# Penguin-jpg/clip-diffusion

Hardware: NVIDIA B200
Metric: CLIP-guided cutouts/s fwd+bwd inside full guidance steps (= steps/s x cutouts per step) @512x512 (higher is better)
Workload: dtype bf16

## Files before the change

clip_diffusion_b200/csrc/vit_attention_tc.cu:

```cuda
#include <stdlib.h>
#include "common.cuh"
#include "tcgen05.cuh"

using namespace tc;

namespace {

constexpr int AT_THREADS = 512;
constexpr int MAX_BLK = 5;
constexpr float LOG2E_F = 1.4426950408889634f;
constexpr uint32_t BLK_BYTES = 64 * 128;
constexpr uint32_t TILE_BYTES = 128 * 128;

__device__ __forceinline__ uint32_t pack_bf2(float a, float b) {
  __nv_bfloat162 v = __floats2bfloat162_rn(a, b);
  return *reinterpret_cast<uint32_t*>(&v);
}
__device__ __forceinline__ float ex2f(float x) {
  float y;
  asm("ex2.approx.ftz.f32 %0, %1;" : "=f"(y) : "f"(x));
  return y;
}
__device__ __forceinline__ float warp_max_f(float v) {
#pragma unroll
  for (int o = 16; o > 0; o >>= 1) v = fmaxf(v, __shfl_xor_sync(0xffffffffu, v, o));
  return v;
}
__device__ __forceinline__ void tmem_ld16(uint32_t taddr, uint32_t* r) {
  asm volatile(
      "tcgen05.ld.sync.aligned.32x32b.x16.b32 {%0, %1, %2, %3, %4, %5, %6, %7, %8, %9, %10, %11, %12, %13, %14, %15}, [%16];"
      : "=r"(r[0]), "=r"(r[1]), "=r"(r[2]), "=r"(r[3]), "=r"(r[4]), "=r"(r[5]), "=r"(r[6]), "=r"(r[7]), "=r"(r[8]), "=r"(r[9]), "=r"(r[10]),
        "=r"(r[11]), "=r"(r[12]), "=r"(r[13]), "=r"(r[14]), "=r"(r[15])
      : "r"(taddr)
      : "memory");
}
__device__ __forceinline__ uint32_t elect_one() {
  uint32_t pred;
  asm volatile("{\n\t.reg .pred P;\n\telect.sync _|P, 0xffffffff;\n\tselp.u32 %0, 1, 0, P;\n\t}" : "=r"(pred));
  return pred;
}
__device__ __forceinline__ uint32_t idesc_bf16(int n, bool b_mn_major) {
  return (1u << 4) | (1u << 7) | (1u << 10) | (b_mn_major ? (1u << 16) : 0u) | ((uint32_t)(n >> 3) << 17) | ((uint32_t)(128 >> 4) << 24);
}
__device__ __forceinline__ void st_shared_v4(uint32_t a, uint32_t x, uint32_t y, uint32_t z, uint32_t w) {
  asm volatile("st.shared.v4.b32 [%0], {%1, %2, %3, %4};" ::"r"(a), "r"(x), "r"(y), "r"(z), "r"(w) : "memory");
}
__device__ __forceinline__ void st256g(void* p, const uint32_t* w) {
  asm volatile("st.global.v8.b32 [%0], {%1,%2,%3,%4,%5,%6,%7,%8};" ::"l"(p), "r"(w[0]), "r"(w[1]), "r"(w[2]), "r"(w[3]), "r"(w[4]), "r"(w[5]),
               "r"(w[6]), "r"(w[7])
               : "memory");
}
__device__ __forceinline__ void store_row64_bf16(__nv_bfloat16* dst, const uint32_t* a, const uint32_t* b, float mul) {
  uint32_t w[32];
#pragma unroll
  for (int j = 0; j < 16; ++j) {
    w[j] = pack_bf2(__uint_as_float(a[2 * j]) * mul, __uint_as_float(a[2 * j + 1]) * mul);
    w[16 + j] = pack_bf2(__uint_as_float(b[2 * j]) * mul, __uint_as_float(b[2 * j + 1]) * mul);
  }
#pragma unroll
  for (int j = 0; j < 4; ++j) st256g(dst + 16 * j, w + 8 * j);
}

__device__ __forceinline__ uint32_t lds32(uint32_t a) {
  uint32_t v;
  asm volatile("ld.shared.b32 %0, [%1];" : "=r"(v) : "r"(a) : "memory");
  return v;
}
__device__ __forceinline__ float bf_lo(uint32_t u) { return __uint_as_float(u << 16); }
__device__ __forceinline__ float bf_hi(uint32_t u) { return __uint_as_float(u & 0xffff0000u); }
__device__ __forceinline__ float dot8p(const uint4 a, const uint4 b, float acc) {
  acc = fmaf(bf_lo(a.x), bf_lo(b.x), acc); acc = fmaf(bf_hi(a.x), bf_hi(b.x), acc); acc = fmaf(bf_lo(a.y), bf_lo(b.y), acc); acc = fmaf(bf_hi(a.y), bf_hi(b.y), acc);
  acc = fmaf(bf_lo(a.z), bf_lo(b.z), acc); acc = fmaf(bf_hi(a.z), bf_hi(b.z), acc); acc = fmaf(bf_lo(a.w), bf_lo(b.w), acc); acc = fmaf(bf_hi(a.w), bf_hi(b.w), acc);
  return acc;
}

struct AttnParams {
  int T, heads, ntiles, nblk, tail_rows;
  int nitems;
  int edge, nblk_ld, ld_tail;
  float scale;
  __nv_bfloat16* ctx;
  float* lse;
  const __nv_bfloat16* ctx_in;
  const __nv_bfloat16* dctx_in;
  __nv_bfloat16* dqkv;
  long long* trace;
};

struct FBars {
  uint32_t base;
  __device__ __forceinline__ uint32_t sfull(int b) const { return base + 8u * b; }
  __device__ __forceinline__ uint32_t sfree(int b) const { return base + 32u + 8u * b; }
  __device__ __forceinline__ uint32_t pready(int b) const { return base + 64u + 8u * b; }
  __device__ __forceinline__ uint32_t pfree(int b) const { return base + 96u + 8u * b; }
  __device__ __forceinline__ uint32_t accfull(int a) const { return base + 128u + 8u * a; }
  __device__ __forceinline__ uint32_t accfree(int a) const { return base + 160u + 8u * a; }
  __device__ __forceinline__ uint32_t mready(int a, uint32_t r) const { return base + 192u + 8u * (2u * a + r); }
  __device__ __forceinline__ uint32_t opq(int blk) const { return base + 256u + 8u * blk; }
  __device__ __forceinline__ uint32_t opk(int blk) const { return base + 296u + 8u * blk; }
  __device__ __forceinline__ uint32_t opv(int vb, int blk) const { return base + 336u + 8u * (vb * MAX_BLK + blk); }
  __device__ __forceinline__ uint32_t qkfree() const { return base + 416u; }
  __device__ __forceinline__ uint32_t vfree(int vb) const { return base + 424u + 8u * vb; }
  __device__ __forceinline__ uint32_t tmem_slot() const { return base + 440u; }
};
constexpr uint32_t FBARS_BYTES = 448 + 16;
constexpr uint32_t FWD_FLOATS = 4096 + 1024;
constexpr float RESCALE_LOG2 = 8.f;

__device__ __forceinline__ void tmem_st32(uint32_t taddr, const uint32_t* r) {
  asm volatile(
      "tcgen05.st.sync.aligned.32x32b.x32.b32 [%0], "
      "{%1, %2, %3, %4, %5, %6, %7, %8, %9, %10, %11, %12, %13, %14, %15, %16, "
      "%17, %18, %19, %20, %21, %22, %23, %24, %25, %26, %27, %28, %29, %30, %31, %32};" ::"r"(taddr),
      "r"(r[0]), "r"(r[1]), "r"(r[2]), "r"(r[3]), "r"(r[4]), "r"(r[5]), "r"(r[6]), "r"(r[7]), "r"(r[8]), "r"(r[9]), "r"(r[10]), "r"(r[11]), "r"(r[12]),
      "r"(r[13]), "r"(r[14]), "r"(r[15]), "r"(r[16]), "r"(r[17]), "r"(r[18]), "r"(r[19]), "r"(r[20]), "r"(r[21]), "r"(r[22]), "r"(r[23]), "r"(r[24]),
      "r"(r[25]), "r"(r[26]), "r"(r[27]), "r"(r[28]), "r"(r[29]), "r"(r[30]), "r"(r[31])
      : "memory");
}
__device__ __forceinline__ void tmem_st16(uint32_t taddr, const uint32_t* r) {
  asm volatile(
      "tcgen05.st.sync.aligned.32x32b.x16.b32 [%0], {%1, %2, %3, %4, %5, %6, %7, %8, %9, %10, %11, %12, %13, %14, %15, %16};" ::"r"(taddr),
      "r"(r[0]), "r"(r[1]), "r"(r[2]), "r"(r[3]), "r"(r[4]), "r"(r[5]), "r"(r[6]), "r"(r[7]), "r"(r[8]), "r"(r[9]), "r"(r[10]), "r"(r[11]), "r"(r[12]),
      "r"(r[13]), "r"(r[14]), "r"(r[15])
      : "memory");
}
// ... 555 lines not shown
      if (lane == 0) mbar_arrive(bars.vfree(vb));
    };
    float se0 = -INFINITY, se1 = -INFINITY, nse0 = -INFINITY, nse1 = -INFINITY;
    if ((int)blockIdx.x < nitems) { edge_a(blockIdx.x, 0, se0, se1); edge_b(blockIdx.x, 0); }
    int it = 0, gg0 = 0;
    for (int w = blockIdx.x; w < nitems; w += gridDim.x, ++it, gg0 += G) {
      const int n = w / heads, h = w - n * heads, row0 = n * T;
      const float* vedge = vedge2 + (it & 1) * 64;
      TRF(warp, 62, 0);
      TRI(warp, 0);
      for (int tile = 0; tile < ntiles; ++tile) {
        const int tp = tile & 1, a0 = tp, a1 = 2 + tp;
        const int ggt = gg0 + tile * nblk;
        const bool has0 = nblk > 1 || (ggt & 1) == 0, has1 = nblk > 1 || (ggt & 1) == 1;
        const uint32_t u0 = (euse >> (4 * a0)) & 15u, u1 = (euse >> (4 * a1)) & 15u;
        if (has0) { mbar_wait(bars.mready(a0, u0 & 1u), (u0 >> 1) & 1u); mbar_wait(bars.accfull(a0), u0 & 1u); }
        if (has1) { mbar_wait(bars.mready(a1, u1 & 1u), (u1 >> 1) & 1u); mbar_wait(bars.accfull(a1), u1 & 1u); }
        TRF(warp, tile, 0);
        tcgen05_fence_after();
        const int row = tile * 128 + rl;
        if (tile * 128 + q * 32 < Tp) {
          const float m0 = has0 ? sm[(a0 * 4 + (int)(u0 & 3u)) * 128 + rl] : -INFINITY, m1 = has1 ? sm[(a1 * 4 + (int)(u1 & 3u)) * 128 + rl] : -INFINITY;
          const float l0 = has0 ? sl[(a0 * 4 + (int)(u0 & 3u)) * 128 + rl] : 0.f, l1 = has1 ? sl[(a1 * 4 + (int)(u1 & 3u)) * 128 + rl] : 0.f;
          const float se = tile == 0 ? se0 : se1;
          const float M = fmaxf(fmaxf(m0, m1), se);
          const float f0 = has0 ? ex2f(m0 - M) : 0.f, f1 = has1 ? ex2f(m1 - M) : 0.f, fe = ex2f(se - M);
          const float L = l0 * f0 + l1 * f1 + fe;
          const float invL = __fdividef(1.f, L);
          const float g0 = f0 * invL, g1 = f1 * invL, ge = fe * invL;
          __nv_bfloat16* dst = p.ctx + ((long long)(row0 + row)) * D + h * 64;
#pragma unroll
          for (int c = 0; c < 64; c += 32) {
            uint32_t v0[32], v1[32], wv[16];
            if (has0) tmem_ld32(t_lane + 256u + (uint32_t)(a0 * 64 + c), v0);
            if (has1) tmem_ld32(t_lane + 256u + (uint32_t)(a1 * 64 + c), v1);
            tmem_ld_wait();
#pragma unroll
            for (int j = 0; j < 16; ++j) {
              float x0 = (has0 ? __uint_as_float(v0[2 * j]) * g0 : 0.f) + (has1 ? __uint_as_float(v1[2 * j]) * g1 : 0.f);
              float x1 = (has0 ? __uint_as_float(v0[2 * j + 1]) * g0 : 0.f) + (has1 ? __uint_as_float(v1[2 * j + 1]) * g1 : 0.f);
              if (edge) {
                const float2 ve = *reinterpret_cast<const float2*>(vedge + c + 2 * j);
                x0 = fmaf(ge, ve.x, x0);
                x1 = fmaf(ge, ve.y, x1);
              }
              wv[j] = pack_bf2(x0, x1);
            }
            if (row < Tp) { st256g(dst + c, wv); st256g(dst + c + 16, wv + 8); }
          }
          if (row < Tp) p.lse[((long long)n * heads + h) * T + row] = M * (1.f / LOG2E_F) + logf(L);
        }
        tcgen05_fence_before();
        __syncwarp();
        if (lane == 0) {
          if (has0) mbar_arrive(bars.accfree(a0));
          if (has1) mbar_arrive(bars.accfree(a1));
        }
        if (has0) euse = (euse & ~(15u << (4 * a0))) | (((u0 + 1u) & 15u) << (4 * a0));
        if (has1) euse = (euse & ~(15u << (4 * a1))) | (((u1 + 1u) & 15u) << (4 * a1));
        TRF(warp, tile, 1);
        if (tile == 0 && w + (int)gridDim.x < nitems) {
          TRF(warp, 61, 0);
          edge_a(w + gridDim.x, it + 1, nse0, nse1);
          edge_b(w + gridDim.x, it + 1);
          TRF(warp, 61, 1);
        }
      }
      se0 = nse0;
      se1 = nse1;
      TRF(warp, 62, 1);
      TRI(warp, 1);
    }
  }
  tcgen05_fence_before();
  __syncthreads();
  if (warp == 2) {
    tcgen05_fence_after();
    asm volatile("tcgen05.dealloc.cta_group::1.sync.aligned.b32 %0, %1;" ::"r"(tmem_base), "r"(512) : "memory");
  }
}

struct BBars {
  uint32_t base;
  __device__ __forceinline__ uint32_t sfull(int b) const { return base + 8u * b; }
  __device__ __forceinline__ uint32_t sfree(int b) const { return base + 24u + 8u * b; }
  __device__ __forceinline__ uint32_t pready(int pb) const { return base + 48u + 8u * pb; }
  __device__ __forceinline__ uint32_t pfree(int pb) const { return base + 64u + 8u * pb; }
  __device__ __forceinline__ uint32_t accfull(int a) const { return base + 80u + 8u * a; }
  __device__ __forceinline__ uint32_t accfree(int a) const { return base + 104u + 8u * a; }
  __device__ __forceinline__ uint32_t op(int o, int blk) const { return base + 128u + 8u * (o * MAX_BLK + blk); }
  __device__ __forceinline__ uint32_t opfree() const { return base + 288u; }
  __device__ __forceinline__ uint32_t cready(int par) const { return base + 296u + 8u * par; }
  __device__ __forceinline__ uint32_t tmem_slot() const { return base + 312u; }
};
constexpr uint32_t BBARS_BYTES = 320 + 16;
constexpr uint32_t BWD_FLOATS = 1280 + 1152 + 192 + 768;

#ifdef CG_ATTN_TRACE
#define TRB(slot, idx, ev) TRF(slot, idx, ev)
#else
#define TRB(slot, idx, ev) do { } while (0)
#endif

__device__ __forceinline__ void store_row64_bf16_axpy(__nv_bfloat16* dst, const uint32_t* a, const uint32_t* b, float coef, const float* vec) {
  uint32_t w[32];
#pragma unroll
  for (int j = 0; j < 16; ++j) {
    const float2 v0 = *reinterpret_cast<const float2*>(vec + 2 * j), v1 = *reinterpret_cast<const float2*>(vec + 32 + 2 * j);
    w[j] = pack_bf2(fmaf(coef, v0.x, __uint_as_float(a[2 * j])), fmaf(coef, v0.y, __uint_as_float(a[2 * j + 1])));
    w[16 + j] = pack_bf2(fmaf(coef, v1.x, __uint_as_float(b[2 * j])), fmaf(coef, v1.y, __uint_as_float(b[2 * j + 1])));
  }
#pragma unroll
  for (int j = 0; j < 4; ++j) st256g(dst + 16 * j, w + 8 * j);
}

__global__ void __launch_bounds__(AT_THREADS, 1)
    attn_bwd_tc_kernel(const __grid_constant__ CUtensorMap tmQKV, const __grid_constant__ CUtensorMap tmQKVtail, const __grid_constant__ CUtensorMap tmDO,
                       const __grid_constant__ CUtensorMap tmDOtail, const AttnParams p) {
  extern __shared__ __align__(1024) uint8_t smem_raw[];
  cg_griddep_launch();
  constexpr int NSB = 3;
  constexpr uint32_t STAGE_BYTES = 2 * TILE_BYTES;
  const int T = p.T, heads = p.heads, D = heads * 64;
  const int edge = p.edge, Tp = T - edge;
  const int warp = threadIdx.x >> 5, lane = threadIdx.x & 31;
  const int ntiles = p.ntiles, nblk = p.nblk, nblk_ld = p.nblk_ld;
  const int per_phase = ntiles * nblk, G = 2 * per_phase, nitems = p.nitems;
  const uint32_t opb = (uint32_t)((nblk_ld - 1) * 64 + p.ld_tail) * 128u;
  const uint32_t base = (smem_u32(smem_raw) + 1023u) & ~1023u;
  const uint32_t sOp0 = base;
  const uint32_t sStage = base + 4 * opb;
  const uint32_t sF = sStage + 2 * STAGE_BYTES;
  float* fscr = reinterpret_cast<float*>(smem_raw + (sF - smem_u32(smem_raw)));
  float* csts = fscr;
  float* ev = fscr + 1280;
  float* evec = fscr + 2432;
  float* epart = fscr + 2624;
  BBars bars{sF + BWD_FLOATS * 4};

  if (warp == 0 && lane == 0) {
    asm volatile("prefetch.tensormap [%0];" ::"l"(&tmQKV) : "memory");
    asm volatile("prefetch.tensormap [%0];" ::"l"(&tmQKVtail) : "memory");
    asm volatile("prefetch.tensormap [%0];" ::"l"(&tmDO) : "memory");
    asm volatile("prefetch.tensormap [%0];" ::"l"(&tmDOtail) : "memory");
    for (int b = 0; b < 3; ++b) {
      mbar_init(bars.sfull(b), 2); mbar_init(bars.sfree(b), 4);
      mbar_init(bars.accfull(b), 2); mbar_init(bars.accfree(b), 4);
    }
    for (int b = 0; b < 2; ++b) { mbar_init(bars.pready(b), 4); mbar_init(bars.pfree(b), 2); mbar_init(bars.cready(b), 4); }
    for (int o = 0; o < 4; ++o)
      for (int k = 0; k < MAX_BLK; ++k) mbar_init(bars.op(o, k), 1);
    mbar_init(bars.opfree(), 8);
    asm volatile("fence.mbarrier_init.release.cluster;" ::: "memory");
  }
  if (warp == 2) {
    asm volatile("tcgen05.alloc.cta_group::1.sync.aligned.shared::cta.b32 [%0], %1;" ::"r"(bars.tmem_slot()), "r"(512) : "memory");
    asm volatile("tcgen05.relinquish_alloc_permit.cta_group::1.sync.aligned;" ::: "memory");
  }
  cg_griddep_wait();
  tcgen05_fence_before();
  __syncthreads();
  tcgen05_fence_after();
  uint32_t tmem_base;
  asm volatile("ld.shared.b32 %0, [%1];" : "=r"(tmem_base) : "r"(bars.tmem_slot()) : "memory");

  if (warp < 4) {
    const uint32_t elected = elect_one();
    const uint32_t id_full = idesc_bf16(64, false), id_tail = idesc_bf16(p.tail_rows, false), id_acc = idesc_bf16(64, true);
    uint32_t cuse = 0;
    int it = 0, gg0 = 0;
    for (int w = blockIdx.x; w < nitems; w += gridDim.x, ++it, gg0 += G) {
      const uint32_t opar = (uint32_t)it & 1u;
      uint32_t loaded = 0;
      auto need = [&](int o, int blk) {
        const uint32_t bit = 1u << (o * MAX_BLK + blk);
        if (!(loaded & bit)) { mbar_wait(bars.op(o, blk), opar); loaded |= bit; }
      };
      if (warp == 3) {
        if (elected) {
          if (it > 0) mbar_wait(bars.opfree(), (uint32_t)(it - 1) & 1u);
          const int n = w / heads, h = w - n * heads, row0 = n * T;
          auto load = [&](int o, int blk) {
            const bool tail = blk == nblk_ld - 1;
            const uint32_t bar = bars.op(o, blk);
            mbar_arrive_expect_tx(bar, (uint32_t)(tail ? p.ld_tail : 64) * 128u);
            if (o < 3) tma_load_2d(sOp0 + o * opb + blk * BLK_BYTES, tail ? &tmQKVtail : &tmQKV, bar, o * D + h * 64, row0 + blk * 64);
            else tma_load_2d(sOp0 + o * opb + blk * BLK_BYTES, tail ? &tmDOtail : &tmDO, bar, h * 64, row0 + blk * 64);
          };
          const int first = nblk_ld < 2 ? nblk_ld : 2;
          load(1, 0);
#pragma unroll 1
          for (int k = 0; k < first; ++k) load(0, k);
          load(2, 0);
#pragma unroll 1
          for (int k = 0; k < first; ++k) load(3, k);
#pragma unroll 1
          for (int k = 1; k < nblk_ld; ++k) { load(1, k); load(2, k); }
#pragma unroll 1
          for (int k = first; k < nblk_ld; ++k) { load(0, k); load(3, k); }
          if (w + (int)gridDim.x < nitems) {
            const int w2 = w + gridDim.x, n2 = w2 / heads, h2 = w2 - n2 * heads;
#pragma unroll 1
            for (int k = 0; k < nblk_ld; ++k) {
              const bool tail = k == nblk_ld - 1;
#pragma unroll 1
              for (int o = 0; o < 3; ++o) tma_prefetch_2d(tail ? &tmQKVtail : &tmQKV, o * D + h2 * 64, n2 * T + k * 64);
              tma_prefetch_2d(tail ? &tmDOtail : &tmDO, h2 * 64, n2 * T + k * 64);
            }
          }
        }
        __syncwarp();
      }
      int phase = 0, tile = 0, blk = 0;
      if (warp < 2) {
        for (int g = 0; g < G; ++g) {
          const int gg = gg0 + g, b = gg % NSB;
          const bool transposed = phase == 1;
          const int oa = warp == 0 ? (transposed ? 1 : 0) : (transposed ? 2 : 3);
          const int ob = warp == 0 ? (transposed ? 0 : 1) : (transposed ? 3 : 2);
          need(oa, 2 * tile);
          if (2 * tile + 1 < nblk) need(oa, 2 * tile + 1);
          need(ob, blk);
          mbar_wait(bars.sfree(b), ((uint32_t)(gg / NSB) & 1u) ^ 1u);
          TRB(warp, g, 0);
          tcgen05_fence_after();
          const uint32_t d_s = tmem_base + (uint32_t)(b * 128) + (warp == 1 ? 64u : 0u);
          const uint64_t ad = make_smem_desc(sOp0 + oa * opb + tile * TILE_BYTES), bd = make_smem_desc(sOp0 + ob * opb + blk * BLK_BYTES);
          const uint32_t idesc = blk == nblk - 1 ? id_tail : id_full;
          if (elected) {
#pragma unroll
            for (int k = 0; k < 4; ++k) umma_bf16(d_s, ad + (uint64_t)(2 * k), bd + (uint64_t)(2 * k), idesc, k != 0 ? 1u : 0u);
            umma_commit(bars.sfull(b));
          }
          __syncwarp();
          TRB(warp, g, 1);
          if (++blk == nblk) { blk = 0; if (++tile == ntiles) { tile = 0; ++phase; } }
        }
      } else {
        const int wi = warp - 2;
        for (int g = 0; g < G; ++g) {
          const int gg = gg0 + g, pb = gg & 1;
          const int a = phase == 1 ? 2 : (tile & 1);
          const bool does_mma = phase == 1 || wi == 0;
          const int ob = phase == 0 ? 1 : (wi == 0 ? 3 : 0);
          if (does_mma) need(ob, blk);
          mbar_wait(bars.pready(pb), (uint32_t)(gg >> 1) & 1u);
          TRB(warp, g, 0);
          if (blk == 0) {
            if (phase == 1) {
              mbar_wait(bars.accfree(2), ((cuse >> 2) & 1u) ^ 1u);
              if (tile == 0) { mbar_wait(bars.accfree(0), (cuse & 1u) ^ 1u); mbar_wait(bars.accfree(1), ((cuse >> 1) & 1u) ^ 1u); }
            } else {
              mbar_wait(bars.accfree(a), ((cuse >> a) & 1u) ^ 1u);
              mbar_wait(bars.accfree(2), ((cuse >> 2) & 1u) ^ 1u);
            }
          }
          tcgen05_fence_after();
          const int ksteps = (blk == nblk - 1 ? p.tail_rows : 64) >> 4;
          const uint32_t stage = sStage + pb * STAGE_BYTES + (wi == 1 ? TILE_BYTES : 0u);
          const uint32_t d_acc = tmem_base + (a == 2 ? 384u : 384u + 64u * a) + (wi == 1 ? 64u : 0u);
          const uint64_t ad = make_smem_desc(stage), bd = make_smem_desc(sOp0 + ob * opb + blk * BLK_BYTES);
          const bool last = blk == nblk - 1;
          if (elected) {
            if (does_mma) {
              for (int k = 0; k < ksteps; ++k) umma_bf16(d_acc, ad + (uint64_t)(2 * k), bd + (uint64_t)(128 * k), id_acc, (blk | k) != 0 ? 1u : 0u);
              umma_commit(bars.pfree(pb));
              if (last) umma_commit(bars.accfull(a));
            } else {
              mbar_arrive(bars.pfree(pb));
              if (last) mbar_arrive(bars.accfull(a));
            }
          }
          __syncwarp();
          TRB(warp, g, 1);
          if (last) cuse ^= 1u << a;
          if (++blk == nblk) { blk = 0; if (++tile == ntiles) { tile = 0; ++phase; } }
        }
      }
#pragma unroll 1
      for (int o = 0; o < 4; ++o)
#pragma unroll 1
        for (int k = 0; k < nblk_ld; ++k) need(o, k);
      if (elected) umma_commit(bars.opfree());
      __syncwarp();
    }
  } else if (warp < 12) {
    const int wg = (warp - 4) >> 2;
    const int q = warp & 3;
    const int rl = q * 32 + lane;
    const uint32_t t_lane = tmem_base + ((uint32_t)(q * 32) << 16);
    const float scale = p.scale, sl2 = p.scale * LOG2E_F;
    const int tail_cols = Tp - (nblk - 1) * 64, tail_cols16 = p.tail_rows;
    const uint32_t sx = (uint32_t)(rl & 7) << 4;
    int it = 0, gg0 = 0;
    for (int w = blockIdx.x; w < nitems; w += gridDim.x, ++it, gg0 += G) {
      mbar_wait(bars.cready(it & 1), (uint32_t)(it >> 1) & 1u);
      const float* cst = csts + (it & 1) * 640;
      float rc0 = 0.f, rc1 = 0.f;
      int phase = 0, tile = 0, blk = wg, cur_tile = -1;
      while (blk >= nblk) { blk -= nblk; if (++tile == ntiles) { tile = 0; ++phase; } }
      for (int g = wg; g < G; g += 2) {
        const int gg = gg0 + g;
        if (phase == 0 && tile != cur_tile) {
          const int row = tile * 128 + rl;
          rc0 = row < Tp ? cst[row] : 0.f;
          rc1 = row < Tp ? cst[320 + row] : 0.f;
          cur_tile = tile;
        }
        const bool wvalid = tile * 128 + q * 32 < Tp;
        const bool tail = blk == nblk - 1;
        const int ncols = tail ? tail_cols : 64, ncols16 = tail ? tail_cols16 : 64;
        const int b = gg % NSB, pb = gg & 1;
        const uint32_t suse = (uint32_t)(gg / NSB), puse = (uint32_t)(gg >> 1);
        TRB(warp, g, 0);
        mbar_wait(bars.sfull(b), suse & 1u);
        TRB(warp, g, 1);
        tcgen05_fence_after();
        const uint32_t t_s = t_lane + (uint32_t)(b * 128);
        const uint32_t stage = sStage + pb * STAGE_BYTES + (uint32_t)rl * 128u;
        if (!wvalid) {
          tcgen05_fence_before();
          __syncwarp();
          if (lane == 0) mbar_arrive(bars.sfree(b));
          mbar_wait(bars.pfree(pb), (puse & 1u) ^ 1u);
        } else {
          uint32_t sv[2][16], dv[2][16], w0[8], w1[8];
          const int npieces = ncols16 >> 4;
          tmem_ld16(t_s, sv[0]);
          tmem_ld16(t_s + 64u, dv[0]);
          tmem_ld_wait();
          bool waited = false;
#pragma unroll
          for (int pc = 0; pc < 4; ++pc) {
            if (pc < npieces) {
              const int cur = pc & 1;
              if (pc + 1 < npieces) {
                tmem_ld16(t_s + (uint32_t)(16 * (pc + 1)), sv[cur ^ 1]);
                tmem_ld16(t_s + 64u + (uint32_t)(16 * (pc + 1)), dv[cur ^ 1]);
              }
              if (phase == 0) {
#pragma unroll
                for (int j = 0; j < 8; ++j) {
                  float p0 = ex2f(fmaf(__uint_as_float(sv[cur][2 * j]), sl2, rc0)), p1 = ex2f(fmaf(__uint_as_float(sv[cur][2 * j + 1]), sl2, rc0));
                  if (tail) { if (16 * pc + 2 * j >= ncols) p0 = 0.f; if (16 * pc + 2 * j + 1 >= ncols) p1 = 0.f; }
                  w0[j] = pack_bf2(p0 * fmaf(__uint_as_float(dv[cur][2 * j]), scale, rc1), p1 * fmaf(__uint_as_float(dv[cur][2 * j + 1]), scale, rc1));
                }
              } else {
                const float* nl = cst + blk * 64 + 16 * pc;
                const float* dl = nl + 320;
#pragma unroll
                for (int j = 0; j < 8; ++j) {
                  const float2 l2 = *reinterpret_cast<const float2*>(nl + 2 * j), d2 = *reinterpret_cast<const float2*>(dl + 2 * j);
                  float p0 = ex2f(fmaf(__uint_as_float(sv[cur][2 * j]), sl2, l2.x)), p1 = ex2f(fmaf(__uint_as_float(sv[cur][2 * j + 1]), sl2, l2.y));
                  if (tail) { if (16 * pc + 2 * j >= ncols) p0 = 0.f; if (16 * pc + 2 * j + 1 >= ncols) p1 = 0.f; }
                  w0[j] = pack_bf2(p0, p1);
                  w1[j] = pack_bf2(p0 * fmaf(__uint_as_float(dv[cur][2 * j]), scale, d2.x), p1 * fmaf(__uint_as_float(dv[cur][2 * j + 1]), scale, d2.y));
                }
              }
              if (!waited) { mbar_wait(bars.pfree(pb), (puse & 1u) ^ 1u); waited = true; }
              {
                const uint32_t c0 = ((uint32_t)(pc * 32)) ^ sx, c1 = ((uint32_t)(pc * 32 + 16)) ^ sx;
                st_shared_v4(stage + c0, w0[0], w0[1], w0[2], w0[3]);
                st_shared_v4(stage + c1, w0[4], w0[5], w0[6], w0[7]);
                if (phase == 1) {
                  st_shared_v4(stage + TILE_BYTES + c0, w1[0], w1[1], w1[2], w1[3]);
                  st_shared_v4(stage + TILE_BYTES + c1, w1[4], w1[5], w1[6], w1[7]);
                }
              }
              if (pc + 1 < npieces) {
                tmem_ld_wait();
              } else {
                tcgen05_fence_before();
                __syncwarp();
                if (lane == 0) mbar_arrive(bars.sfree(b));
              }
            }
          }
        }
        TRB(warp, g, 2);
        fence_proxy_async_smem();
        __syncwarp();
        if (lane == 0) mbar_arrive(bars.pready(pb));
        TRB(warp, g, 3);
        blk += 2;
        while (blk >= nblk) { blk -= nblk; if (++tile == ntiles) { tile = 0; ++phase; } }
      }
    }
  } else {
    const int q = warp & 3;
    const int rl = q * 32 + lane;
    const uint32_t t_lane = tmem_base + ((uint32_t)(q * 32) << 16);
    const float scale = p.scale, sl2 = p.scale * LOG2E_F;
    uint32_t euse = 0;
    auto load_consts = [&](int item, int par) {
      const int n = item / heads, h = item - n * heads;
      const float* lb = p.lse + ((long long)n * heads + h) * T;
      const __nv_bfloat16* ob = p.ctx_in + ((long long)n * T) * D + h * 64;
      const __nv_bfloat16* gb = p.dctx_in + ((long long)n * T) * D + h * 64;
      float* c = csts + par * 640;
      for (int i = rl; i < 320; i += 128) {
        float dl = 0.f, nl = -INFINITY;
        if (i < T) {
          const uint4* o4 = reinterpret_cast<const uint4*>(ob + (long long)i * D);
          const uint4* g4 = reinterpret_cast<const uint4*>(gb + (long long)i * D);
          uint4 xo[8], xg[8];
#pragma unroll
          for (int k = 0; k < 8; ++k) { xo[k] = __ldg(o4 + k); xg[k] = __ldg(g4 + k); }
          float d0 = 0.f, d1 = 0.f;
#pragma unroll
          for (int k = 0; k < 8; k += 2) { d0 = dot8p(xo[k], xg[k], d0); d1 = dot8p(xo[k + 1], xg[k + 1], d1); }
          dl = d0 + d1;
          nl = -lb[i] * LOG2E_F;
        }
        c[i] = nl;
        c[320 + i] = -p.scale * dl;
      }
      __syncwarp();
      if (lane == 0) mbar_arrive(bars.cready(par));
    };
    if ((int)blockIdx.x < nitems) load_consts(blockIdx.x, 0);
    int it = 0;
    for (int w = blockIdx.x; w < nitems; w += gridDim.x, ++it) {
      const int n = w / heads, h = w - n * heads, row0 = n * T;
      const uint32_t opar = (uint32_t)it & 1u;
      if (w + (int)gridDim.x < nitems) load_consts(w + gridDim.x, (it + 1) & 1);
      const float* cst = csts + (it & 1) * 640;
      __nv_bfloat16* out = p.dqkv + ((long long)row0) * 3 * D + h * 64;
      TRB(warp, 62, 0);
      TRI(warp, 0);
      if (edge) {
        for (int o = 0; o < 4; ++o)
          for (int k = 0; k < nblk_ld; ++k) mbar_wait(bars.op(o, k), opar);
        mbar_wait(bars.cready(it & 1), (uint32_t)(it >> 1) & 1u);
        TRB(warp, 61, 0);
        const uint32_t sQ = sOp0, sK = sOp0 + opb, sV = sOp0 + 2 * opb, sDO = sOp0 + 3 * opb;
        const float nle = cst[Tp], dle = cst[320 + Tp];
        const int g = lane >> 2, t = lane & 3;
        {
          uint32_t vbk[8], vbv[8], vbq[8], vbd[8];
          load_vec_bfrag(sK, Tp, vbk);
          load_vec_bfrag(sV, Tp, vbv);
          load_vec_bfrag(sQ, Tp, vbq);
          load_vec_bfrag(sDO, Tp, vbd);
#pragma unroll 1
          for (int rg = q; rg < (Tp >> 4); rg += 4) {
            const float2 s_c = mv16(sQ, rg * 16, vbk), dp_c = mv16(sDO, rg * 16, vbv), s_r = mv16(sK, rg * 16, vbq), dp_r = mv16(sV, rg * 16, vbd);
            if (t == 0) {
#pragma unroll
              for (int hh = 0; hh < 2; ++hh) {
                const int i = rg * 16 + g + 8 * hh;
                const float p_c = ex2f(fmaf(hh ? s_c.y : s_c.x, sl2, cst[i]));
                ev[i] = p_c;
                ev[288 + i] = p_c * fmaf(hh ? dp_c.y : dp_c.x, scale, cst[320 + i]);
                const float p_r = ex2f(fmaf(hh ? s_r.y : s_r.x, sl2, nle));
                ev[576 + i] = p_r;
                ev[864 + i] = p_r * fmaf(hh ? dp_r.y : dp_r.x, scale, dle);
              }
            }
          }
        }
        {
          const uint32_t eo = (uint32_t)Tp * 128u + (uint32_t)lane * 4u;
          const uint32_t wq = lds32(sQ + eo), wk = lds32(sK + eo), wv = lds32(sV + eo), wd = lds32(sDO + eo);
          const float s_e = warp_sum(fmaf(bf_lo(wq), bf_lo(wk), bf_hi(wq) * bf_hi(wk)));
          const float dp_e = warp_sum(fmaf(bf_lo(wd), bf_lo(wv), bf_hi(wd) * bf_hi(wv)));
          const float p_e = ex2f(fmaf(s_e, sl2, nle)), ds_e = p_e * fmaf(dp_e, scale, dle);
          if (rl == 0) { ev[Tp] = p_e; ev[288 + Tp] = ds_e; ev[576 + Tp] = p_e; ev[864 + Tp] = ds_e; }
          if (rl >= 1 && rl < 16) { ev[Tp + rl] = 0.f; ev[288 + Tp + rl] = 0.f; ev[576 + Tp + rl] = 0.f; ev[864 + Tp + rl] = 0.f; }
          if (q == 0) {
            evec[2 * lane] = bf_lo(wk); evec[2 * lane + 1] = bf_hi(wk);
            evec[64 + 2 * lane] = bf_lo(wq); evec[64 + 2 * lane + 1] = bf_hi(wq);
            evec[128 + 2 * lane] = bf_lo(wd); evec[128 + 2 * lane + 1] = bf_hi(wd);
          }
        }
        asm volatile("bar.sync 2, 128;" ::: "memory");
        {
          const int ngrp = (Tp >> 4) + 1;
#pragma unroll 1
          for (int pr = 0; pr < 3; ++pr) {
            const uint32_t buf = pr == 0 ? sK : (pr == 1 ? sQ : sDO);
            const float* vec = ev + (pr == 0 ? 864 : (pr == 1 ? 288 : 0));
            float acc[8][4];
#pragma unroll
            for (int nn = 0; nn < 8; ++nn) acc[nn][0] = acc[nn][1] = acc[nn][2] = acc[nn][3] = 0.f;
#pragma unroll 1
            for (int ks = q; ks < ngrp; ks += 4) vm16(buf, ks * 16, vec, acc);
            if (lane < 4) {
#pragma unroll
              for (int nn = 0; nn < 8; ++nn) *reinterpret_cast<float2*>(epart + (pr * 4 + q) * 64 + 8 * nn + 2 * t) = make_float2(acc[nn][0], acc[nn][1]);
            }
          }
          asm volatile("bar.sync 2, 128;" ::: "memory");
          if (q < 3) {
            const float* pp = epart + q * 256 + 2 * lane;
            const float2 x0 = *reinterpret_cast<const float2*>(pp), x1 = *reinterpret_cast<const float2*>(pp + 64);
            const float2 x2 = *reinterpret_cast<const float2*>(pp + 128), x3 = *reinterpret_cast<const float2*>(pp + 192);
            reinterpret_cast<uint32_t*>(out + (long long)Tp * 3 * D + q * D)[lane] = pack_bf2((x0.x + x1.x) + (x2.x + x3.x), (x0.y + x1.y) + (x2.y + x3.y));
          }
        }
        TRB(warp, 61, 1);
      }
      __syncwarp();
      if (lane == 0) mbar_arrive(bars.opfree());
      for (int tc = 0; tc < 2 * ntiles; ++tc) {
        const int phase = tc >= ntiles ? 1 : 0, tile = tc - phase * ntiles;
        const int a = phase == 1 ? 2 : (tile & 1);
        const int row = tile * 128 + rl;
        mbar_wait(bars.accfull(a), (euse >> a) & 1u);
        TRB(warp, tc, 0);
        tcgen05_fence_after();
        if (tile * 128 + q * 32 < Tp) {
          uint32_t v0[32], v1[32];
          const uint32_t col = a == 2 ? 384u : 384u + 64u * a;
          tmem_ld32(t_lane + col, v0);
          tmem_ld32(t_lane + col + 32u, v1);
          tmem_ld_wait();
          __nv_bfloat16* orow = out + (long long)row * 3 * D;
          if (phase == 0) {
            if (row < Tp) {
              if (edge) store_row64_bf16_axpy(orow, v0, v1, ev[288 + row], evec);
              else store_row64_bf16(orow, v0, v1, 1.f);
            }
          } else {
            if (row < Tp) {
              if (edge) store_row64_bf16_axpy(orow + 2 * D, v0, v1, ev[576 + row], evec + 128);
              else store_row64_bf16(orow + 2 * D, v0, v1, 1.f);
            }
            tmem_ld32(t_lane + col + 64u, v0);
            tmem_ld32(t_lane + col + 96u, v1);
            tmem_ld_wait();
            if (row < Tp) {
              if (edge) store_row64_bf16_axpy(orow + D, v0, v1, ev[864 + row], evec + 64);
              else store_row64_bf16(orow + D, v0, v1, 1.f);
            }
          }
        }
        tcgen05_fence_before();
        __syncwarp();
        if (lane == 0) mbar_arrive(bars.accfree(a));
        euse ^= 1u << a;
        TRB(warp, tc, 1);
      }
      TRB(warp, 62, 1);
      TRI(warp, 1);
    }
  }
  tcgen05_fence_before();
  __syncthreads();
  if (warp == 2) {
    tcgen05_fence_after();
    asm volatile("tcgen05.dealloc.cta_group::1.sync.aligned.b32 %0, %1;" ::"r"(tmem_base), "r"(512) : "memory");
  }
}

long long* g_trace = nullptr;

int edge_env() {
  static int v = -1;
  if (v < 0) {
    const char* e = getenv("CG_ATTN_EDGE");
    v = e ? atoi(e) : 3;
  }
  return v;
}
bool fwd_edge_enabled() { return (edge_env() & 1) != 0; }
bool bwd_edge_enabled() { return (edge_env() & 2) != 0; }
void set_geometry(AttnParams& p, int T, bool allow_edge) {
  p.edge = (allow_edge && T > 1 && (T - 1) % 64 == 0) ? 1 : 0;
  const int Tp = T - p.edge;
  p.ntiles = (Tp + 127) / 128;
  p.nblk = (Tp + 63) / 64;
  p.tail_rows = ((Tp - (p.nblk - 1) * 64) + 15) & ~15;
  p.nblk_ld = p.nblk + p.edge;
  p.ld_tail = p.edge ? 16 : p.tail_rows;
}

int cg_num_sms() {
  static int per_device[CG_MAX_DEVICES] = {};
  const int dev = cg_device_index();
  if (per_device[dev] == 0) {
    int n = 0;
    cudaDeviceGetAttribute(&n, cudaDevAttrMultiProcessorCount, dev);
    per_device[dev] = n > 0 ? n : CG_NUM_SMS;
  }
  return per_device[dev];
}

int tc_enabled() {
  static int enabled = -1;
  if (enabled < 0) {
    const char* e = getenv("CG_ATTN_TC");
    enabled = e ? (atoi(e) != 0) : 1;
  }
  return enabled;
}

int launch_attn_bwd_tc(const void* qkv, const void* dctx, int Nimg, int T, int heads, const AttnParams& p0, cudaStream_t s) {
  AttnParams p = p0;
  p.T = T; p.heads = heads; p.scale = 0.125f;
  p.trace = g_trace;
  set_geometry(p, T, bwd_edge_enabled());
  const int D = heads * 64;
  CUtensorMap tq, tqt, td, tdt;
  int rc = cg_make_tensor_map_bf16(&tq, qkv, (long long)Nimg * T, 3LL * D, 3LL * D, 64);
  if (rc) return rc;
  rc = cg_make_tensor_map_bf16(&tqt, qkv, (long long)Nimg * T, 3LL * D, 3LL * D, p.ld_tail);
  if (rc) return rc;
  rc = cg_make_tensor_map_bf16(&td, dctx, (long long)Nimg * T, D, D, 64);
  if (rc) return rc;
  rc = cg_make_tensor_map_bf16(&tdt, dctx, (long long)Nimg * T, D, D, p.ld_tail);
  if (rc) return rc;
  const size_t opb = (size_t)((p.nblk_ld - 1) * 64 + p.ld_tail) * 128;
  const size_t smem = 1024 + 4 * opb + 4 * (size_t)TILE_BYTES + BWD_FLOATS * 4 + BBARS_BYTES;
  p.nitems = Nimg * heads;
  const int grid = p.nitems < cg_num_sms() ? p.nitems : cg_num_sms();
  static size_t configured[CG_MAX_DEVICES] = {};
  const int dev = cg_device_index();
  if (smem > configured[dev]) {
    CG_CUDA(cudaFuncSetAttribute(attn_bwd_tc_kernel, cudaFuncAttributeMaxDynamicSharedMemorySize, (int)smem));
    configured[dev] = smem;
  }
  CG_CUDA(cg_launch_pdl(attn_bwd_tc_kernel, dim3(grid), dim3(AT_THREADS), smem, s, tq, tqt, td, tdt, p));
  return 0;
}

// ... 53 lines not shown
```

Baseline: 1397.

## Fuse attention backward into single pass computing dQ alongside dK/dV

```diff
diff --git a/clip_diffusion_b200/csrc/vit_attention_tc.cu b/clip_diffusion_b200/csrc/vit_attention_tc.cu
--- a/clip_diffusion_b200/csrc/vit_attention_tc.cu
+++ b/clip_diffusion_b200/csrc/vit_attention_tc.cu
@@ -39,8 +39,9 @@
   asm volatile("{\n\t.reg .pred P;\n\telect.sync _|P, 0xffffffff;\n\tselp.u32 %0, 1, 0, P;\n\t}" : "=r"(pred));
   return pred;
 }
-__device__ __forceinline__ uint32_t idesc_bf16(int n, bool b_mn_major) {
-  return (1u << 4) | (1u << 7) | (1u << 10) | (b_mn_major ? (1u << 16) : 0u) | ((uint32_t)(n >> 3) << 17) | ((uint32_t)(128 >> 4) << 24);
+__device__ __forceinline__ uint32_t idesc_bf16(int n, bool b_mn_major, int m = 128, bool a_mn_major = false) {
+  return (1u << 4) | (1u << 7) | (1u << 10) | (a_mn_major ? (1u << 15) : 0u) | (b_mn_major ? (1u << 16) : 0u) | ((uint32_t)(n >> 3) << 17) |
+         ((uint32_t)(m >> 4) << 24);
 }
 __device__ __forceinline__ void st_shared_v4(uint32_t a, uint32_t x, uint32_t y, uint32_t z, uint32_t w) {
   asm volatile("st.shared.v4.b32 [%0], {%1, %2, %3, %4};" ::"r"(a), "r"(x), "r"(y), "r"(z), "r"(w) : "memory");
@@ -762,12 +763,14 @@
 
 struct BBars {
   uint32_t base;
-  __device__ __forceinline__ uint32_t sfull(int b) const { return base + 8u * b; }
-  __device__ __forceinline__ uint32_t sfree(int b) const { return base + 24u + 8u * b; }
-  __device__ __forceinline__ uint32_t pready(int pb) const { return base + 48u + 8u * pb; }
-  __device__ __forceinline__ uint32_t pfree(int pb) const { return base + 64u + 8u * pb; }
-  __device__ __forceinline__ uint32_t accfull(int a) const { return base + 80u + 8u * a; }
-  __device__ __forceinline__ uint32_t accfree(int a) const { return base + 104u + 8u * a; }
+  __device__ __forceinline__ uint32_t sfull(int w) const { return base + 8u * w; }
+  __device__ __forceinline__ uint32_t sfree(int w) const { return base + 16u + 8u * w; }
+  __device__ __forceinline__ uint32_t pready(int pb) const { return base + 32u + 8u * pb; }
+  __device__ __forceinline__ uint32_t pfree(int pb) const { return base + 48u + 8u * pb; }
+  __device__ __forceinline__ uint32_t kvfull() const { return base + 64u; }
+  __device__ __forceinline__ uint32_t kvfree() const { return base + 72u; }
+  __device__ __forceinline__ uint32_t dqfull(int r) const { return base + 80u + 8u * r; }
+  __device__ __forceinline__ uint32_t dqfree(int r) const { return base + 104u + 8u * r; }
   __device__ __forceinline__ uint32_t op(int o, int blk) const { return base + 128u + 8u * (o * MAX_BLK + blk); }
   __device__ __forceinline__ uint32_t opfree() const { return base + 288u; }
   __device__ __forceinline__ uint32_t cready(int par) const { return base + 296u + 8u * par; }
@@ -799,13 +802,14 @@
                        const __grid_constant__ CUtensorMap tmDOtail, const AttnParams p) {
   extern __shared__ __align__(1024) uint8_t smem_raw[];
   cg_griddep_launch();
-  constexpr int NSB = 3;
   constexpr uint32_t STAGE_BYTES = 2 * TILE_BYTES;
   const int T = p.T, heads = p.heads, D = heads * 64;
   const int edge = p.edge, Tp = T - edge;
   const int warp = threadIdx.x >> 5, lane = threadIdx.x & 31;
   const int ntiles = p.ntiles, nblk = p.nblk, nblk_ld = p.nblk_ld;
-  const int per_phase = ntiles * nblk, G = 2 * per_phase, nitems = p.nitems;
+  const int G = ntiles * nblk, nitems = p.nitems;
+  const int nsb = nblk > 4 ? 1 : 2;
+  const uint32_t col_kv = 128u * (uint32_t)nsb, col_dq = col_kv + 128u;
   const uint32_t opb = (uint32_t)((nblk_ld - 1) * 64 + p.ld_tail) * 128u;
   const uint32_t base = (smem_u32(smem_raw) + 1023u) & ~1023u;
   const uint32_t sOp0 = base;
@@ -823,11 +827,12 @@
     asm volatile("prefetch.tensormap [%0];" ::"l"(&tmQKVtail) : "memory");
     asm volatile("prefetch.tensormap [%0];" ::"l"(&tmDO) : "memory");
     asm volatile("prefetch.tensormap [%0];" ::"l"(&tmDOtail) : "memory");
-    for (int b = 0; b < 3; ++b) {
+    for (int b = 0; b < 2; ++b) {
       mbar_init(bars.sfull(b), 2); mbar_init(bars.sfree(b), 4);
-      mbar_init(bars.accfull(b), 2); mbar_init(bars.accfree(b), 4);
+      mbar_init(bars.pready(b), 4); mbar_init(bars.pfree(b), 2); mbar_init(bars.cready(b), 4);
     }
-    for (int b = 0; b < 2; ++b) { mbar_init(bars.pready(b), 4); mbar_init(bars.pfree(b), 2); mbar_init(bars.cready(b), 4); }
+    mbar_init(bars.kvfull(), 2); mbar_init(bars.kvfree(), 4);
+    for (int r = 0; r < 3; ++r) { mbar_init(bars.dqfull(r), 1); mbar_init(bars.dqfree(r), 4); }
     for (int o = 0; o < 4; ++o)
       for (int k = 0; k < MAX_BLK; ++k) mbar_init(bars.op(o, k), 1);
     mbar_init(bars.opfree(), 8);
@@ -847,7 +852,7 @@
   if (warp < 4) {
     const uint32_t elected = elect_one();
     const uint32_t id_full = idesc_bf16(64, false), id_tail = idesc_bf16(p.tail_rows, false), id_acc = idesc_bf16(64, true);
-    uint32_t cuse = 0;
+    const uint32_t id_dq = idesc_bf16(64, true, 64, true);
     int it = 0, gg0 = 0;
     for (int w = blockIdx.x; w < nitems; w += gridDim.x, ++it, gg0 += G) {
       const uint32_t opar = (uint32_t)it & 1u;
@@ -868,16 +873,16 @@
             else tma_load_2d(sOp0 + o * opb + blk * BLK_BYTES, tail ? &tmDOtail : &tmDO, bar, h * 64, row0 + blk * 64);
           };
           const int first = nblk_ld < 2 ? nblk_ld : 2;
-          load(1, 0);
-#pragma unroll 1
-          for (int k = 0; k < first; ++k) load(0, k);
-          load(2, 0);
-#pragma unroll 1
-          for (int k = 0; k < first; ++k) load(3, k);
-#pragma unroll 1
-          for (int k = 1; k < nblk_ld; ++k) { load(1, k); load(2, k); }
-#pragma unroll 1
-          for (int k = first; k < nblk_ld; ++k) { load(0, k); load(3, k); }
+#pragma unroll 1
+          for (int k = 0; k < first; ++k) load(1, k);
+          load(0, 0);
+#pragma unroll 1
+          for (int k = 0; k < first; ++k) load(2, k);
+          load(3, 0);
+#pragma unroll 1
+          for (int k = 1; k < nblk_ld; ++k) { load(0, k); load(3, k); }
+#pragma unroll 1
+          for (int k = first; k < nblk_ld; ++k) { load(1, k); load(2, k); }
           if (w + (int)gridDim.x < nitems) {
             const int w2 = w + gridDim.x, n2 = w2 / heads, h2 = w2 - n2 * heads;
 #pragma unroll 1
@@ -891,70 +896,67 @@
         }
         __syncwarp();
       }
-      int phase = 0, tile = 0, blk = 0;
+      int kt = 0, qb = 0;
       if (warp < 2) {
+        const int oa = warp == 0 ? 1 : 2, ob = warp == 0 ? 0 : 3;
         for (int g = 0; g < G; ++g) {
-          const int gg = gg0 + g, b = gg % NSB;
-          const bool transposed = phase == 1;
-          const int oa = warp == 0 ? (transposed ? 1 : 0) : (transposed ? 2 : 3);
-          const int ob = warp == 0 ? (transposed ? 0 : 1) : (transposed ? 3 : 2);
-          need(oa, 2 * tile);
-          if (2 * tile + 1 < nblk) need(oa, 2 * tile + 1);
-          need(ob, blk);
-          mbar_wait(bars.sfree(b), ((uint32_t)(gg / NSB) & 1u) ^ 1u);
+          const int gg = gg0 + g, prev = gg - nsb;
+          need(oa, 2 * kt);
+          if (2 * kt + 1 < nblk) need(oa, 2 * kt + 1);
+          need(ob, qb);
+          if (prev >= 0) mbar_wait(bars.sfree(prev & 1), (uint32_t)(prev >> 1) & 1u);
           TRB(warp, g, 0);
           tcgen05_fence_after();
-          const uint32_t d_s = tmem_base + (uint32_t)(b * 128) + (warp == 1 ? 64u : 0u);
-          const uint64_t ad = make_smem_desc(sOp0 + oa * opb + tile * TILE_BYTES), bd = make_smem_desc(sOp0 + ob * opb + blk * BLK_BYTES);
-          const uint32_t idesc = blk == nblk - 1 ? id_tail : id_full;
+          const uint32_t d_s = tmem_base + (uint32_t)((gg % nsb) * 128) + (warp == 1 ? 64u : 0u);
+          const uint64_t ad = make_smem_desc(sOp0 + oa * opb + kt * TILE_BYTES), bd = make_smem_desc(sOp0 + ob * opb + qb * BLK_BYTES);
+          const uint32_t idesc = qb == nblk - 1 ? id_tail : id_full;
           if (elected) {
 #pragma unroll
             for (int k = 0; k < 4; ++k) umma_bf16(d_s, ad + (uint64_t)(2 * k), bd + (uint64_t)(2 * k), idesc, k != 0 ? 1u : 0u);
-            umma_commit(bars.sfull(b));
+            umma_commit(bars.sfull(gg & 1));
           }
           __syncwarp();
           TRB(warp, g, 1);
-          if (++blk == nblk) { blk = 0; if (++tile == ntiles) { tile = 0; ++phase; } }
+          if (++qb == nblk) { qb = 0; ++kt; }
         }
       } else {
         const int wi = warp - 2;
+        const int ob = wi == 0 ? 3 : 0;
         for (int g = 0; g < G; ++g) {
           const int gg = gg0 + g, pb = gg & 1;
-          const int a = phase == 1 ? 2 : (tile & 1);
-          const bool does_mma = phase == 1 || wi == 0;
-          const int ob = phase == 0 ? 1 : (wi == 0 ? 3 : 0);
-          if (does_mma) need(ob, blk);
+          need(ob, qb);
+          if (wi == 0) { need(1, 2 * kt); if (2 * kt + 1 < nblk) need(1, 2 * kt + 1); }
           mbar_wait(bars.pready(pb), (uint32_t)(gg >> 1) & 1u);
           TRB(warp, g, 0);
-          if (blk == 0) {
-            if (phase == 1) {
-              mbar_wait(bars.accfree(2), ((cuse >> 2) & 1u) ^ 1u);
-              if (tile == 0) { mbar_wait(bars.accfree(0), (cuse & 1u) ^ 1u); mbar_wait(bars.accfree(1), ((cuse >> 1) & 1u) ^ 1u); }
-            } else {
-              mbar_wait(bars.accfree(a), ((cuse >> a) & 1u) ^ 1u);
-              mbar_wait(bars.accfree(2), ((cuse >> 2) & 1u) ^ 1u);
+          if (qb == 0) mbar_wait(bars.kvfree(), (uint32_t)(it * ntiles + kt + 1) & 1u);
+          tcgen05_fence_after();
+          const int ksteps = (qb == nblk - 1 ? p.tail_rows : 64) >> 4;
+          const uint32_t stage = sStage + pb * STAGE_BYTES;
+          const uint32_t d_acc = tmem_base + col_kv + (wi == 1 ? 64u : 0u);
+          const uint64_t ad = make_smem_desc(stage + (wi == 1 ? TILE_BYTES : 0u)), bd = make_smem_desc(sOp0 + ob * opb + qb * BLK_BYTES);
+          const bool last_q = qb == nblk - 1;
+          if (elected)
+            for (int k = 0; k < ksteps; ++k) umma_bf16(d_acc, ad + (uint64_t)(2 * k), bd + (uint64_t)(128 * k), id_acc, (qb | k) != 0 ? 1u : 0u);
+          if (wi == 0) {
+            if (kt == 0 && !(qb & 1)) {
+              mbar_wait(bars.dqfree(qb >> 1), opar ^ 1u);
+              tcgen05_fence_after();
             }
-          }
-          tcgen05_fence_after();
-          const int ksteps = (blk == nblk - 1 ? p.tail_rows : 64) >> 4;
-          const uint32_t stage = sStage + pb * STAGE_BYTES + (wi == 1 ? TILE_BYTES : 0u);
-          const uint32_t d_acc = tmem_base + (a == 2 ? 384u : 384u + 64u * a) + (wi == 1 ? 64u : 0u);
-          const uint64_t ad = make_smem_desc(stage), bd = make_smem_desc(sOp0 + ob * opb + blk * BLK_BYTES);
-          const bool last = blk == nblk - 1;
+            const int keys = Tp - 128 * kt < 128 ? Tp - 128 * kt : 128, kq = (keys + 15) >> 4;
+            const uint32_t d_q = tmem_base + col_dq + 64u * (uint32_t)(qb >> 1) + ((uint32_t)(16 * (qb & 1)) << 16);
+            const uint64_t aq = make_smem_desc(stage + TILE_BYTES), bq = make_smem_desc(sOp0 + opb + kt * TILE_BYTES);
+            if (elected) {
+              for (int k = 0; k < kq; ++k) umma_bf16(d_q, aq + (uint64_t)(128 * k), bq + (uint64_t)(128 * k), id_dq, (kt | k) != 0 ? 1u : 0u);
+              if (kt == ntiles - 1 && ((qb & 1) || last_q)) umma_commit(bars.dqfull(qb >> 1));
+            }
+          }
           if (elected) {
-            if (does_mma) {
-              for (int k = 0; k < ksteps; ++k) umma_bf16(d_acc, ad + (uint64_t)(2 * k), bd + (uint64_t)(128 * k), id_acc, (blk | k) != 0 ? 1u : 0u);
-              umma_commit(bars.pfree(pb));
-              if (last) umma_commit(bars.accfull(a));
-            } else {
-              mbar_arrive(bars.pfree(pb));
-              if (last) mbar_arrive(bars.accfull(a));
-            }
+            umma_commit(bars.pfree(pb));
+            if (last_q) umma_commit(bars.kvfull());
           }
           __syncwarp();
           TRB(warp, g, 1);
-          if (last) cuse ^= 1u << a;
-          if (++blk == nblk) { blk = 0; if (++tile == ntiles) { tile = 0; ++phase; } }
+          if (++qb == nblk) { qb = 0; ++kt; }
         }
       }
 #pragma unroll 1
@@ -968,47 +970,44 @@
     const int wg = (warp - 4) >> 2;
     const int q = warp & 3;
     const int rl = q * 32 + lane;
-    const uint32_t t_lane = tmem_base + ((uint32_t)(q * 32) << 16);
+    const uint32_t t_s = tmem_base + ((uint32_t)(q * 32) << 16) + (nsb == 2 ? 128u * (uint32_t)wg : 0u);
+    const uint32_t stage = sStage + (uint32_t)wg * STAGE_BYTES + (uint32_t)rl * 128u;
     const float scale = p.scale, sl2 = p.scale * LOG2E_F;
     const int tail_cols = Tp - (nblk - 1) * 64, tail_cols16 = p.tail_rows;
     const uint32_t sx = (uint32_t)(rl & 7) << 4;
+    auto release_s = [&]() {
+      tcgen05_fence_before();
+      __syncwarp();
+      if (lane == 0) mbar_arrive(bars.sfree(wg));
+    };
     int it = 0, gg0 = 0;
     for (int w = blockIdx.x; w < nitems; w += gridDim.x, ++it, gg0 += G) {
+      int g = (wg ^ gg0) & 1;
+      if (g >= G) continue;
       mbar_wait(bars.cready(it & 1), (uint32_t)(it >> 1) & 1u);
       const float* cst = csts + (it & 1) * 640;
-      float rc0 = 0.f, rc1 = 0.f;
-      int phase = 0, tile = 0, blk = wg, cur_tile = -1;
-      while (blk >= nblk) { blk -= nblk; if (++tile == ntiles) { tile = 0; ++phase; } }
-      for (int g = wg; g < G; g += 2) {
+      int kt = g / nblk, qb = g - kt * nblk;
+      for (; g < G; g += 2) {
         const int gg = gg0 + g;
-        if (phase == 0 && tile != cur_tile) {
-          const int row = tile * 128 + rl;
-          rc0 = row < Tp ? cst[row] : 0.f;
-          rc1 = row < Tp ? cst[320 + row] : 0.f;
-          cur_tile = tile;
-        }
-        const bool wvalid = tile * 128 + q * 32 < Tp;
-        const bool tail = blk == nblk - 1;
+        const uint32_t use = (uint32_t)(gg >> 1);
+        const bool wvalid = kt * 128 + q * 32 < Tp;
+        const bool kvalid = kt * 128 + rl < Tp;
+        const bool tail = qb == nblk - 1;
         const int ncols = tail ? tail_cols : 64, ncols16 = tail ? tail_cols16 : 64;
-        const int b = gg % NSB, pb = gg & 1;
-        const uint32_t suse = (uint32_t)(gg / NSB), puse = (uint32_t)(gg >> 1);
         TRB(warp, g, 0);
-        mbar_wait(bars.sfull(b), suse & 1u);
+        mbar_wait(bars.sfull(wg), use & 1u);
         TRB(warp, g, 1);
         tcgen05_fence_after();
-        const uint32_t t_s = t_lane + (uint32_t)(b * 128);
-        const uint32_t stage = sStage + pb * STAGE_BYTES + (uint32_t)rl * 128u;
         if (!wvalid) {
-          tcgen05_fence_before();
-          __syncwarp();
-          if (lane == 0) mbar_arrive(bars.sfree(b));
-          mbar_wait(bars.pfree(pb), (puse & 1u) ^ 1u);
+          release_s();
+          mbar_wait(bars.pfree(wg), (use & 1u) ^ 1u);
         } else {
           uint32_t sv[2][16], dv[2][16], w0[8], w1[8];
           const int npieces = ncols16 >> 4;
           tmem_ld16(t_s, sv[0]);
           tmem_ld16(t_s + 64u, dv[0]);
           tmem_ld_wait();
+          if (npieces == 1) release_s();
           bool waited = false;
 #pragma unroll
           for (int pc = 0; pc < 4; ++pc) {
@@ -1018,41 +1017,27 @@
                 tmem_ld16(t_s + (uint32_t)(16 * (pc + 1)), sv[cur ^ 1]);
                 tmem_ld16(t_s + 64u + (uint32_t)(16 * (pc + 1)), dv[cur ^ 1]);
               }
-              if (phase == 0) {
-#pragma unroll
-                for (int j = 0; j < 8; ++j) {
-                  float p0 = ex2f(fmaf(__uint_as_float(sv[cur][2 * j]), sl2, rc0)), p1 = ex2f(fmaf(__uint_as_float(sv[cur][2 * j + 1]), sl2, rc0));
-                  if (tail) { if (16 * pc + 2 * j >= ncols) p0 = 0.f; if (16 * pc + 2 * j + 1 >= ncols) p1 = 0.f; }
-                  w0[j] = pack_bf2(p0 * fmaf(__uint_as_float(dv[cur][2 * j]), scale, rc1), p1 * fmaf(__uint_as_float(dv[cur][2 * j + 1]), scale, rc1));
-                }
-              } else {
-                const float* nl = cst + blk * 64 + 16 * pc;
-                const float* dl = nl + 320;
-#pragma unroll
-                for (int j = 0; j < 8; ++j) {
-                  const float2 l2 = *reinterpret_cast<const float2*>(nl + 2 * j), d2 = *reinterpret_cast<const float2*>(dl + 2 * j);
-                  float p0 = ex2f(fmaf(__uint_as_float(sv[cur][2 * j]), sl2, l2.x)), p1 = ex2f(fmaf(__uint_as_float(sv[cur][2 * j + 1]), sl2, l2.y));
-                  if (tail) { if (16 * pc + 2 * j >= ncols) p0 = 0.f; if (16 * pc + 2 * j + 1 >= ncols) p1 = 0.f; }
-                  w0[j] = pack_bf2(p0, p1);
-                  w1[j] = pack_bf2(p0 * fmaf(__uint_as_float(dv[cur][2 * j]), scale, d2.x), p1 * fmaf(__uint_as_float(dv[cur][2 * j + 1]), scale, d2.y));
-                }
+              const float* nl = cst + qb * 64 + 16 * pc;
+              const float* dl = nl + 320;
+#pragma unroll
+              for (int j = 0; j < 8; ++j) {
+                const float2 l2 = *reinterpret_cast<const float2*>(nl + 2 * j), d2 = *reinterpret_cast<const float2*>(dl + 2 * j);
+                float p0 = ex2f(fmaf(__uint_as_float(sv[cur][2 * j]), sl2, l2.x)), p1 = ex2f(fmaf(__uint_as_float(sv[cur][2 * j + 1]), sl2, l2.y));
+                if (tail) { if (16 * pc + 2 * j >= ncols) p0 = 0.f; if (16 * pc + 2 * j + 1 >= ncols) p1 = 0.f; }
+                w0[j] = pack_bf2(p0, p1);
+                w1[j] = kvalid ? pack_bf2(p0 * fmaf(__uint_as_float(dv[cur][2 * j]), scale, d2.x), p1 * fmaf(__uint_as_float(dv[cur][2 * j + 1]), scale, d2.y)) : 0u;
               }
-              if (!waited) { mbar_wait(bars.pfree(pb), (puse & 1u) ^ 1u); waited = true; }
+              if (!waited) { mbar_wait(bars.pfree(wg), (use & 1u) ^ 1u); waited = true; }
               {
                 const uint32_t c0 = ((uint32_t)(pc * 32)) ^ sx, c1 = ((uint32_t)(pc * 32 + 16)) ^ sx;
                 st_shared_v4(stage + c0, w0[0], w0[1], w0[2], w0[3]);
                 st_shared_v4(stage + c1, w0[4], w0[5], w0[6], w0[7]);
-                if (phase == 1) {
-                  st_shared_v4(stage + TILE_BYTES + c0, w1[0], w1[1], w1[2], w1[3]);
-                  st_shared_v4(stage + TILE_BYTES + c1, w1[4], w1[5], w1[6], w1[7]);
-                }
+                st_shared_v4(stage + TILE_BYTES + c0, w1[0], w1[1], w1[2], w1[3]);
+                st_shared_v4(stage + TILE_BYTES + c1, w1[4], w1[5], w1[6], w1[7]);
               }
               if (pc + 1 < npieces) {
                 tmem_ld_wait();
-              } else {
-                tcgen05_fence_before();
-                __syncwarp();
-                if (lane == 0) mbar_arrive(bars.sfree(b));
+                if (pc + 2 == npieces) release_s();
               }
             }
           }
@@ -1060,10 +1045,10 @@
         TRB(warp, g, 2);
         fence_proxy_async_smem();
         __syncwarp();
-        if (lane == 0) mbar_arrive(bars.pready(pb));
+        if (lane == 0) mbar_arrive(bars.pready(wg));
         TRB(warp, g, 3);
-        blk += 2;
-        while (blk >= nblk) { blk -= nblk; if (++tile == ntiles) { tile = 0; ++phase; } }
+        qb += 2;
+        while (qb >= nblk) { qb -= nblk; ++kt; }
       }
     }
   } else {
@@ -1071,7 +1056,6 @@
     const int rl = q * 32 + lane;
     const uint32_t t_lane = tmem_base + ((uint32_t)(q * 32) << 16);
     const float scale = p.scale, sl2 = p.scale * LOG2E_F;
-    uint32_t euse = 0;
     auto load_consts = [&](int item, int par) {
       const int n = item / heads, h = item - n * heads;
       const float* lb = p.lse + ((long long)n * heads + h) * T;
@@ -1182,45 +1166,60 @@
       }
       __syncwarp();
       if (lane == 0) mbar_arrive(bars.opfree());
-      for (int tc = 0; tc < 2 * ntiles; ++tc) {
-        const int phase = tc >= ntiles ? 1 : 0, tile = tc - phase * ntiles;
-        const int a = phase == 1 ? 2 : (tile & 1);
-        const int row = tile * 128 + rl;
-        mbar_wait(bars.accfull(a), (euse >> a) & 1u);
-        TRB(warp, tc, 0);
+      auto drain_kv = [&](int kt) {
+        mbar_wait(bars.kvfull(), (uint32_t)(it * ntiles + kt) & 1u);
+        TRB(warp, kt, 0);
         tcgen05_fence_after();
-        if (tile * 128 + q * 32 < Tp) {
+        const int row = kt * 128 + rl;
+        if (kt * 128 + q * 32 < Tp) {
           uint32_t v0[32], v1[32];
-          const uint32_t col = a == 2 ? 384u : 384u + 64u * a;
-          tmem_ld32(t_lane + col, v0);
-          tmem_ld32(t_lane + col + 32u, v1);
+          __nv_bfloat16* orow = out + (long long)row * 3 * D;
+          tmem_ld32(t_lane + col_kv, v0);
+          tmem_ld32(t_lane + col_kv + 32u, v1);
           tmem_ld_wait();
-          __nv_bfloat16* orow = out + (long long)row * 3 * D;
-          if (phase == 0) {
-            if (row < Tp) {
-              if (edge) store_row64_bf16_axpy(orow, v0, v1, ev[288 + row], evec);
-              else store_row64_bf16(orow, v0, v1, 1.f);
-            }
-          } else {
-            if (row < Tp) {
-              if (edge) store_row64_bf16_axpy(orow + 2 * D, v0, v1, ev[576 + row], evec + 128);
-              else store_row64_bf16(orow + 2 * D, v0, v1, 1.f);
-            }
-            tmem_ld32(t_lane + col + 64u, v0);
-            tmem_ld32(t_lane + col + 96u, v1);
-            tmem_ld_wait();
-            if (row < Tp) {
-              if (edge) store_row64_bf16_axpy(orow + D, v0, v1, ev[864 + row], evec + 64);
-              else store_row64_bf16(orow + D, v0, v1, 1.f);
-            }
+          if (row < Tp) {
+            if (edge) store_row64_bf16_axpy(orow + 2 * D, v0, v1, ev[576 + row], evec + 128);
+            else store_row64_bf16(orow + 2 * D, v0, v1, 1.f);
+          }
+          tmem_ld32(t_lane + col_kv + 64u, v0);
+          tmem_ld32(t_lane + col_kv + 96u, v1);
+          tmem_ld_wait();
+          if (row < Tp) {
+            if (edge) store_row64_bf16_axpy(orow + D, v0, v1, ev[864 + row], evec + 64);
+            else store_row64_bf16(orow + D, v0, v1, 1.f);
           }
         }
         tcgen05_fence_before();
         __syncwarp();
-        if (lane == 0) mbar_arrive(bars.accfree(a));
-        euse ^= 1u << a;
-        TRB(warp, tc, 1);
-      }
+        if (lane == 0) mbar_arrive(bars.kvfree());
+        TRB(warp, kt, 1);
+      };
+      auto drain_dq = [&](int r) {
+        mbar_wait(bars.dqfull(r), opar);
+        TRB(warp, 8 + r, 0);
+        tcgen05_fence_after();
+        uint32_t v0[32], v1[32];
+        tmem_ld32(t_lane + col_dq + 64u * (uint32_t)r, v0);
+        tmem_ld32(t_lane + col_dq + 64u * (uint32_t)r + 32u, v1);
+        tmem_ld_wait();
+        const int qb = 2 * r + (lane >> 4), row = qb * 64 + 16 * q + (lane & 15);
+        if (qb < nblk && row < Tp) {
+          __nv_bfloat16* orow = out + (long long)row * 3 * D;
+          if (edge) store_row64_bf16_axpy(orow, v0, v1, ev[288 + row], evec);
+          else store_row64_bf16(orow, v0, v1, 1.f);
+        }
+        tcgen05_fence_before();
+        __syncwarp();
+        if (lane == 0) mbar_arrive(bars.dqfree(r));
+        TRB(warp, 8 + r, 1);
+      };
+      const int ndq = (nblk + 1) >> 1;
+      for (int kt = 0; kt < ntiles; ++kt) {
+        if (kt == ntiles - 1)
+          for (int r = 0; r + 1 < ndq; ++r) drain_dq(r);
+        drain_kv(kt);
+      }
+      drain_dq(ndq - 1);
       TRB(warp, 62, 1);
       TRI(warp, 1);
     }
```

New measurement: 1422, median of 6. 1.8% higher.
